# Stalfoes/dqn_mgsc_zoo

Measured on AMD Instinct MI355X. Metric: learner grad-steps/sec at batch=32, 84×84×4 uint8, 1/2/4/8 MI355X, higher is better.
Workload: dtype f32

## Files before the change

### dqn_mgsc_zoo_amd/_native.py

```python

import ctypes
import glob
import hashlib
import os
import threading

_HERE = os.path.dirname(os.path.abspath(__file__))
LIB_PATH = os.environ.get('DQZ_LIB') or os.path.join(_HERE, 'libdqz.so')
HEADER_PATH = os.path.join(os.path.dirname(_HERE), 'include', 'dqz.h')

DQZ_OK = 0
ALGO_DQN = 0
ALGO_DOUBLE = 1
ALGO_PER = 2
NUM_LEAVES = 10
NUM_PHASES = 10
PHASE_NAMES = (
    'conv1_fwd', 'conv2_fwd', 'conv3_fwd', 'fc1_fwd', 'head', 'fc1_dx',
    'conv3_dx+conv2_dx+fc1_dw+conv3_dw+conv2_dw+conv1_dw', 'unused7',
    'unused8', 'update')
FRAME_H = 84
FRAME_W = 84
STACK = 4
FRAME_BYTES = FRAME_H * FRAME_W
# ... 210 lines not shown
        [_vp, ctypes.POINTER(DqzParams), ctypes.POINTER(DqzStore), _i64, _i64,
         _i64, ctypes.c_uint64, _vp, _vp, _vp, _vp, _vp]),
    'dqz_learner_step_opt_per_draw': (
        _int,
        [_vp, ctypes.POINTER(DqzParams), ctypes.POINTER(DqzStore),
         ctypes.POINTER(DqzPerDraw), _vp, _vp, _vp]),
    'dqz_learner_grad': (
        _int,
        [_vp, ctypes.POINTER(DqzParams), ctypes.POINTER(DqzStore), _vp, _vp,
         _vp, _vp],
    ),
    'dqz_learner_outputs': (_int, [_vp, _vp, _vp, _vp, _vp]),
    'dqz_learner_sync_status': (_int, [_vp, _vp]),
    'dqz_learner_debug_stall': (_int, [_vp, _int, ctypes.c_uint]),
    'dqz_learner_debug_backward': (_int, [_vp, _int, _vp]),
    'dqz_learner_debug_sync_words': (_int, [_vp, _vp, _i64, _vp]),
    'dqz_learner_debug_activations': (_int, [_vp, _int] + [_vp] * 10),
    'dqz_per_write_back': (_int, [_vp, _vp, _i64, _vp, ctypes.c_double, _vp, _vp]),
    'dqz_learner_profile': (
        _int,
        [_vp, ctypes.POINTER(DqzParams), ctypes.POINTER(DqzStore), _vp, _vp,
         _int, ctypes.POINTER(ctypes.c_float), _vp],
    ),
    'dqz_forward': (_int, [_vp, _vp, _vp, _int, _vp, _vp]),
    'dqz_forward_slots': (
        _int, [_vp, _vp, ctypes.POINTER(DqzStore), _vp, _int, _int, _vp, _vp]),
    'dqz_act': (
        _int, [_vp, _vp, _vp, _int, ctypes.c_double, ctypes.c_uint64,
               ctypes.c_uint64, _vp, _vp]),
    'dqz_store_put': (
# ... 257 lines not shown
```

### dqn_mgsc_zoo_amd/csrc/common.hpp

```cpp
#pragma once
#include <hip/hip_runtime.h>

#include <cstdarg>
#include <cstdint>
#include <cstdio>
#include <string>

#include "dqz.h"

namespace dqz {

typedef float f32x4 __attribute__((ext_vector_type(4)));

#define DQZ_STR(x) #x
#define DQZ_XSTR(x) DQZ_STR(x)
typedef float f32x16 __attribute__((ext_vector_type(16)));

#ifdef DQZ_STEP_TU
#define DQZ_STEP_KERNEL __global__
#define DQZ_OTHER_KERNEL template <int = 0> __global__
#else
#define DQZ_STEP_KERNEL template <int = 0> __global__
#define DQZ_OTHER_KERNEL __global__
#endif
// ... 100 lines not shown
    const float w = 2.f * u * (-lr) * rs3 * (d2 - c1 * g * (g - m));
    nu = w;
    sq += u * u;
    s1 += gq * w;
  }
  __device__ __forceinline__ float meta2(float g, float m0, float v0, float j, float& sq) const {
    const float m = c1 * g + decay * m0;
    const float v = c1 * (g * g) + decay * v0;
    const float u = (-lr) * (g * rsqrtf(v - m * m + eps));
    sq += u * u;
    return -2.f * u * j;
  }
};

#ifdef DQZ_TRACE
constexpr int TRACE_KERNELS = 24, TRACE_BLOCKS = 4096, TRACE_SLOTS = 4;
static __device__ unsigned long long g_dqz_trace[TRACE_KERNELS * TRACE_BLOCKS * TRACE_SLOTS];
#define DQZ_STAMP(kid, slot)                                                                              \
  do {                                                                                                    \
    if (threadIdx.x == 0) {                                                                               \
      const unsigned bl_ = blockIdx.x + gridDim.x * (blockIdx.y + gridDim.y * blockIdx.z);                \
      if (bl_ < (unsigned)dqz::TRACE_BLOCKS)                                                              \
        dqz::g_dqz_trace[((kid) * dqz::TRACE_BLOCKS + bl_) * dqz::TRACE_SLOTS + (slot)] =                \
            __builtin_amdgcn_s_memrealtime();                                                             \
    }                                                                                                     \
  } while (0)
#else
#define DQZ_STAMP(kid, slot) \
  do {                       \
  } while (0)
#endif
// ... 108 lines not shown
  }
  __device__ __forceinline__ void release_finish(int b, int prior, [[maybe_unused]] int hk = -1) const {
    __builtin_amdgcn_sched_barrier(0);
    if (threadIdx.x == 0 && prior == consumers - 1) {
      __hip_atomic_store(cnt + b * kStride, 0, __ATOMIC_RELAXED, __HIP_MEMORY_SCOPE_AGENT);
      __hip_atomic_store(ack + b * kStride, 0, __ATOMIC_RELAXED, __HIP_MEMORY_SCOPE_AGENT);
    }
    if (hk >= 0) DQZ_STAMP(hk, 3);
  }
  __device__ __forceinline__ void wait_release(int b) const {
    wait(b);
    release_finish(b, release_issue(b));
  }
};

constexpr int kTraceY1 = 20, kTraceY2 = 21, kTraceDy2 = 22, kTraceDy1 = 23;

__device__ __forceinline__ float4 load_sc1_f4(const float4* base, int bytes, int e) {
  typedef unsigned u32x4 __attribute__((ext_vector_type(4)));
  const __amdgpu_buffer_rsrc_t r = __builtin_amdgcn_make_buffer_rsrc((void*)base, 0, bytes, 0x00020000);
  return __builtin_bit_cast(float4, __builtin_amdgcn_raw_buffer_load_b128(r, e * 16, 0, 16));
}

__device__ __forceinline__ float load_sc1_f1(const float* base, int bytes, int e) {
  const __amdgpu_buffer_rsrc_t r = __builtin_amdgcn_make_buffer_rsrc((void*)base, 0, bytes, 0x00020000);
  return __builtin_bit_cast(float, __builtin_amdgcn_raw_buffer_load_b32(r, e * 4, 0, 16));
}

__device__ __forceinline__ void store_sc1_f4(float* base, int bytes, int off, f32x4 v) {
  typedef unsigned u32x4 __attribute__((ext_vector_type(4)));
  const __amdgpu_buffer_rsrc_t r = __builtin_amdgcn_make_buffer_rsrc((void*)base, 0, bytes, 0x00020000);
// ... 26 lines not shown
```

### dqn_mgsc_zoo_amd/csrc/fwd.hpp

```cpp
#pragma once
#include "common.hpp"
#include "conv1.hpp"

namespace dqz {


__device__ __forceinline__ f32x4 mfma4(float a, float b, f32x4 c) {
  return __builtin_amdgcn_mfma_f32_16x16x4f32(a, b, c, 0, 0, 0);
}

__device__ __forceinline__ int red_idx(int row, int col) { return row * 16 + 16 * (row >> 2) + col; }

__device__ __forceinline__ int epi_row(int i) {
  return ((i >> 6) << 4) + (int)((0xFBAE9DC873261540ull >> (4 * ((i >> 2) & 15))) & 15);
}
constexpr int epi_range(int rows) { return (rows + 15) / 16 * 64; }
constexpr int red_rows(int rows) { return rows * 16 + 16 * ((rows + 3) / 4); }

struct LayerFwdArgs {
  const float* in;
  NetZ nz;
  int64_t w_off, b_off;
  int B, Z;
  int linear;
// ... 429 lines not shown
}

constexpr int FC1_S = 7, FC1_KS = FLAT / FC1_S, FC1_KW = FC1_KS / 4;
constexpr int Z_MAX_FC1 = 3;

struct Fc1FwdArgs {
  const float* in;
  NetZ nz;
  int64_t w_off;
  int B, MG;
  float* part;
  TangentDot dot = {nullptr, nullptr, 0};
};

constexpr int FC1_32RW = 32 * 33;
template <bool DOT>
__device__ __forceinline__ void fc1_fwd_block32(const Fc1FwdArgs& a, float* s_red, int i) {
  const int nt = i % (HID / 32);
  const int rest = i / (HID / 32);
  const int s = rest % FC1_S, zm = rest / FC1_S;
  const int z = zm / a.MG, mg = zm % a.MG;
  const int t = threadIdx.x, lane = t & 63, w = t >> 6;
  const int c = lane & 31, h = lane >> 5;
  const int k0 = s * FC1_KS + w * FC1_KW + 4 * h;
  const float* W = a.nz.p[z] + a.w_off + 32 * nt + c;
  constexpr int G = FC1_KW / 8;
  const int row = min(32 * mg + c, a.B - 1);
  const float* x = a.in + ((int64_t)z * a.B + row) * FLAT + k0;
  float wr[G][4];
  float4 av[G];
#pragma unroll
  for (int g = 0; g < G; ++g)
// ... 21 lines not shown
    v[e] = (s_red[k] + s_red[FC1_32RW + k]) + (s_red[2 * FC1_32RW + k] + s_red[3 * FC1_32RW + k]);
  }
  if (DOT) {
    float d = 0.f;
    if (live) {
      const float4 dz = *reinterpret_cast<const float4*>(a.dot.dy + (int64_t)(32 * mg + q) * HID + 32 * nt + c4);
      d = (v[0] * dz.x + v[1] * dz.y) + (v[2] * dz.z + v[3] * dz.w);
    }
    d += __shfl_xor(d, 1, 64);
    d += __shfl_xor(d, 2, 64);
    d += __shfl_xor(d, 4, 64);
    if (live && (t & 7) == 0)
      a.dot.part[(int64_t)(32 * mg + q) * META_DOT_SLOTS + a.dot.slot0 + nt * FC1_S + s] = d;
    return;
  }
  if (live)
    *reinterpret_cast<float4*>(a.part + (((int64_t)z * FC1_S + s) * a.B + 32 * mg + q) * HID + 32 * nt + c4) =
        make_float4(v[0], v[1], v[2], v[3]);
}

inline int fc1_fwd_blocks(int Z, int MG) { return (HID / 32) * FC1_S * Z * MG; }

constexpr int FC1_GEMV_MAXB = 4, FC1_GEMV_KG = FC1_KS / 8;
constexpr int FC1_GEMV_SMEM = FC1_GEMV_MAXB * FC1_KS + 8 * FC1_GEMV_MAXB * 32;
__device__ __forceinline__ void fc1_gemv_block(const Fc1FwdArgs& a, float* smem, int i) {
  const int nt = i % (HID / 32);
  const int rest = i / (HID / 32);
  const int s = rest % FC1_S, z = rest / FC1_S;
  const int t = threadIdx.x, c = t & 31, kg = t >> 5;
  const int B = a.B;
// ... 53 lines not shown
```

### dqn_mgsc_zoo_amd/csrc/head.hpp

```cpp
#pragma once
#include "common.hpp"

namespace dqz {

struct HeadArgs {
  const float* fc1p;
  int S;
  float* h1;
  NetZ nz;
  int64_t b1_off, w2_off, b2_off;
  int Z, B, A, algo, shared_bias, fwd_only;
  const int32_t* slots;
  const int32_t* action;
  const float* reward;
  const float* discount;
  const float* weights;
  const double* per_wb;
  int per_normalize;
  float* per_w_out;
  const float* meta_p;
  const float* meta_logits;
  const int32_t* meta_pos;
  int meta_M;
  float *meta_x_out, *meta_p_out;
// ... 32 lines not shown
  return dqz_action{act, v};
}

__device__ __forceinline__ double wave_max_nonneg(double m) {
  m = fmax(m, dpp_d<0x111>(m));
  m = fmax(m, dpp_d<0x112>(m));
  m = fmax(m, dpp_d<0x114>(m));
  m = fmax(m, dpp_d<0x118>(m));
  m = fmax(m, dpp_d<0x142, 0xa>(m));
  m = fmax(m, dpp_d<0x143, 0xc>(m));
  const long long b = __builtin_bit_cast(long long, m);
  const int lo = __builtin_amdgcn_readlane((int)b, 63), hi = __builtin_amdgcn_readlane((int)(b >> 32), 63);
  return __builtin_bit_cast(double, ((long long)hi << 32) | (unsigned)lo);
}

template <int AMAX, int SMAX, int ZMAX>
__device__ __forceinline__ void head_body(const HeadArgs& h, int b, bool out = true, float* s_dzo = nullptr) {
  DQZ_STAMP(4, 0);
  __shared__ float s_red[8][3 * AMAX];
  __shared__ float s_q[3][AMAX];
  __shared__ float s_rec[5];
  const int n = threadIdx.x, lane = n & 63, wave = n >> 6;
  const int A = h.A, B = h.B, Z = h.Z, S = h.S;
  int a_tm1 = 0;
  float r = 0.f, d = 0.f, w = 1.f, pm = 0.f;
  const bool chain = !h.fwd_only && h.rec == nullptr;
  const int slot = chain ? h.slots[b] : 0;
  float4 rv = make_float4(0.f, 0.f, 0.f, 0.f);
  if (!h.fwd_only && h.rec != nullptr && n == 0) rv = h.rec[b];
  float pv[ZMAX][SMAX], b1v[ZMAX], w2v[ZMAX][AMAX];
#pragma unroll
  for (int z = 0; z < ZMAX; ++z) {
    const int zc = min(z, Z - 1);
    const float* part = h.fc1p + ((int64_t)zc * S * B + b) * HID + n;
#pragma unroll
    for (int s = 0; s < SMAX; ++s) pv[z][s] = part[(int64_t)min(s, S - 1) * B * HID];
    b1v[z] = h.nz.p[zc][h.b1_off + n];
    const float* w2 = h.nz.p[zc] + h.w2_off + n * A;
#pragma unroll
    for (int a = 0; a < AMAX; ++a) w2v[z][a] = w2[min(a, A - 1)];
  }
  constexpr bool kTr = AMAX <= 8;
  constexpr int kPS = HID + 16;
  __shared__ float s_p[kTr ? 3 * AMAX : 1][kTr ? kPS : 1];
  const int K = Z * A, lgT = K <= 16 ? 5 : 4, T = 1 << lgT;
  const int kk = n >> lgT, jj = n & (T - 1);
  const bool qthread = kTr ? (kk < K && jj == 0) : (n < 3 * AMAX && n / AMAX < Z && n % AMAX < A);
  const int zq = kTr ? min(kk / A, 2) : n / AMAX, aq = kTr ? kk % A : n % AMAX;
  float b2v = 0.f;
  {
    const int a2 = h.shared_bias ? 0 : min(aq, A - 1);
    float b2z[ZMAX];
#pragma unroll
    for (int z = 0; z < ZMAX; ++z) b2z[z] = h.nz.p[min(z, Z - 1)][h.b2_off + a2];
    const int zc = min(zq, Z - 1);
#pragma unroll
    for (int z = 0; z < ZMAX; ++z) b2v = zc == z ? b2z[z] : b2v;
  }
  float wper = 1.f;
// ... 41 lines not shown
      d = h.discount[slot];
    } else {
      a_tm1 = __float_as_int(rv.x);
      r = rv.y;
      d = rv.z;
    }
    if (h.weights) w = h.weights[b];
    if (h.per_wb) w = wper;
    if (h.meta_p && !h.meta_logits) pm = h.meta_p[b];
    s_rec[0] = __int_as_float(a_tm1);
    s_rec[1] = r;
    s_rec[2] = d;
    s_rec[3] = w;
    s_rec[4] = pm;
  }
  DQZ_STAMP(4, 1);
  float hz[ZMAX];
#pragma unroll
  for (int z = 0; z < ZMAX; ++z) hz[z] = 0.f;
#pragma unroll
  for (int z = 0; z < ZMAX; ++z) {
    if (z < Z) {
      float acc = b1v[z];
#pragma unroll
      for (int s = 0; s < SMAX; ++s) acc += s < S ? pv[z][s] : 0.f;
      hz[z] = relu(acc);
      if (z == 0) DQZ_STAMP(15, 0);
      if constexpr (kTr) {
#pragma unroll
        for (int a = 0; a < AMAX; ++a)
          if (a < A) s_p[z * A + a][n] = hz[z] * w2v[z][a];
      } else {
#pragma unroll
        for (int a = 0; a < AMAX; ++a) {
          const float sa = wave_sum(hz[z] * w2v[z][a]);
          if (lane == 0) s_red[wave][z * AMAX + a] = sa;
        }
      }
    }
  }
  DQZ_STAMP(15, 1);
  __syncthreads();
  float qv = 0.f;
  if constexpr (kTr) {
    if (kk < K) {
      const float* row = &s_p[kk][jj];
      float a4[4] = {0.f, 0.f, 0.f, 0.f};
      for (int i = 0; i < (HID >> lgT); i += 4) {
#pragma unroll
        for (int u = 0; u < 4; ++u) a4[u] += row[(i + u) << lgT];
      }
      float v = (a4[0] + a4[1]) + (a4[2] + a4[3]);
      v += dpp_f<0xB1>(v);
      v += dpp_f<0x4E>(v);
      v += dpp_f<0x141>(v);
      v += dpp_f<0x140>(v);
      if (T == 32) v += __shfl_xor(v, 16, 64);
      qv = v + b2v;
      if (jj == 0) s_q[zq][aq] = qv;
    }
  } else if (qthread) {
// ... 60 lines not shown
      for (int a = 1; a < AMAX; ++a) wv = a == a_tm1 ? w2v[0][a] : wv;
      DQZ_STAMP(4, 2);
      const float dz = hz[0] > 0.f ? -g * wv : 0.f;
      if (s_dzo) s_dzo[n] = dz;
      if (out) h.dz1[(int64_t)b * HID + n] = dz;
    }
  } else if (h.act_out) {
    __syncthreads();
    if (out && n == 0) {
      const uint4 r = philox4x32(make_uint4((unsigned)h.act_ctr, (unsigned)(h.act_ctr >> 32), (unsigned)b, 0xAC7u),
                                 make_uint2((unsigned)h.act_seed, (unsigned)(h.act_seed >> 32)));
      const double u = ((((uint64_t)r.x << 32) | r.y) >> 11) * 0x1.0p-53;
      h.act_out[b] = eps_greedy(s_q[0], A, h.eps, u);
    }
  }
  if (!out) return;
#pragma unroll
  for (int z = 0; z < ZMAX; ++z)
    if (z < Z) h.h1[((int64_t)z * B + b) * HID + n] = hz[z];
  if (qthread) h.q[((int64_t)zq * B + b) * A + aq] = qv;
  if (h.advance && b == 0 && n == 0)
    __hip_atomic_fetch_add(h.advance, (uint64_t)1, __ATOMIC_RELAXED, __HIP_MEMORY_SCOPE_AGENT);
  DQZ_STAMP(4, 3);
}

template <int AMAX, int SMAX, int ZMAX>
__global__ __launch_bounds__(512) void head_kernel(HeadArgs h) {
  head_body<AMAX, SMAX, ZMAX>(h, blockIdx.x);
}

// ... 2 lines not shown
inline void launch_head_z(const HeadArgs& h, int grid, hipStream_t st) {
  if (h.A <= 8)
    hipLaunchKernelGGL((head_kernel<8, SMAX, ZMAX>), dim3(grid), dim3(HID), 0, st, h);
  else
    hipLaunchKernelGGL((head_kernel<MAXA, SMAX, ZMAX>), dim3(grid), dim3(HID), 0, st, h);
}

inline hipError_t launch_head(const HeadArgs& h, int grid, hipStream_t st) {
  if (h.S > 7 || h.Z < 1 || h.Z > 3) return hipErrorInvalidValue;
  if (h.Z <= 2) {
    launch_head_z<7, 2>(h, grid, st);
  } else {
    launch_head_z<7, 3>(h, grid, st);
  }
  return hipGetLastError();
}
#endif

struct UpdArgs {
  float *th, *mu, *nu;
  int64_t off[10];
  int64_t sz[10];
  const float* p1;
  const float* p2;
  const float* p3;
  int S1, S2, S3;
  const float* h1;
  const float* dz1;
  const float* gq;
  const int32_t* ga;
// ... 316 lines not shown
```

### dqn_mgsc_zoo_amd/csrc/layout.hpp

```cpp
#pragma once
#include <cstddef>
#include <cstdint>

namespace dqz {

constexpr int kWordStride = 64;

struct HandoffWords {
  int64_t cnt, ack;
  int need, consumers;
  bool learner_spin;
};

struct SyncLayout {
  int64_t B;
  constexpr int64_t word(int64_t w) const { return w * kWordStride; }
  constexpr HandoffWords dy2() const { return {word(0), word(B), 8, 16, true}; }
  constexpr HandoffWords fwd_y1(int jobs) const { return {word(2 * B), word(5 * B), 4, jobs, false}; }
  constexpr HandoffWords fwd_y2(int jobs) const { return {word(8 * B), word(11 * B), jobs, jobs, false}; }
  constexpr HandoffWords dy1() const { return {word(14 * B), word(15 * B), 8, 8, true}; }
  constexpr int64_t err() const { return word(16 * B); }
  constexpr int64_t ints() const { return word(16 * B + 3) + 64; }
};

enum MetaWord {
  kMetaReseed,
  kMetaDdot1Cnt,
  kMetaDdot1Ack,
  kMetaAdamEntry,
  kMetaErr,
  kMetaWords
};

struct Carve {
  void** pp;
  int64_t n;
  template <class T>
// ... 15 lines not shown
```

### dqn_mgsc_zoo_amd/csrc/learner_impl.hpp

```cpp
#pragma once
#include <hip/hip_runtime.h>

#include <cstring>

#include "common.hpp"
#include "layout.hpp"
#include "conv1.hpp"
#include "fwd.hpp"
#include "head.hpp"
#include "bwd.hpp"
#include "sampling.hpp"

namespace dqz {

inline void param_layout(int A, int shared_bias, int64_t off[10], int64_t sz[10], int64_t* total) {
  const int64_t sizes[10] = {C1KK * C1CO, C1CO, C2KK * C2CO, C2CO, C3KK * C3CO, C3CO,
                             (int64_t)FLAT * HID, HID, (int64_t)HID * A, shared_bias ? 1 : A};
  int64_t o = 0;
  for (int i = 0; i < 10; ++i) {
    off[i] = o;
    sz[i] = sizes[i];
    o += (sizes[i] + 63) / 64 * 64;
  }
  *total = o;
// ... 1 lines not shown

}

struct dqz_learner {
  dqz_learner_config cfg;
  int Z, shared_bias;
  int64_t off[10], sz[10], total;
  int S_fc1, S2, S3;
  float *y1, *y2, *y3, *fc1p, *h1, *q, *dz1, *dy3, *dy2, *dy1, *p1, *p2, *p3, *td, *loss, *loss_part, *gq, *rec;
  float *w3p, *w2p;
  double* per_wb;
  int32_t* ga;
  int32_t* sync;
  unsigned spin_max = 1u << 24;
  int bwd_chain = -1;
  void* block;
};

namespace dqz {

static_assert(Handoff::kStride == kWordStride, "layout.hpp's word stride is Handoff's");

inline SyncLayout sync_of(const dqz_learner* L) { return SyncLayout{L->cfg.batch}; }
inline Handoff handoff(const dqz_learner* L, const HandoffWords& w) {
  Handoff h{L->sync + w.cnt, L->sync + w.ack, L->sync + sync_of(L).err(), w.need, w.consumers};
  if (w.learner_spin) h.spin_max = L->spin_max;
  return h;
}

inline bool bwd_chain_active(const dqz_learner* L) {
  if (L->cfg.batch > BWD_CHAIN_MAXB) return false;
  return L->bwd_chain < 0 ? L->cfg.batch > 1 : L->bwd_chain != 0;
}

inline int check_store(const dqz_store* S) {
  if (!S || !S->frames || !S->fidx || !S->action || !S->reward || !S->discount)
    return fail(DQZ_ERR_INVALID, "store has a null buffer");
  if (S->capacity < 1) return fail(DQZ_ERR_INVALID, "store capacity must be positive");
  return DQZ_OK;
}

inline int device_view(const void* p, const void** out, const char* what) {
  hipPointerAttribute_t attr;
  if (hipPointerGetAttributes(&attr, p) != hipSuccess) {
    (void)hipGetLastError();
    return fail(DQZ_ERR_INVALID, "%s must be device memory or pinned host memory", what);
  }
// ... 219 lines not shown
```

### dqn_mgsc_zoo_amd/csrc/learner_step.hip

```cpp
#define DQZ_STEP_TU 1
#include <hip/hip_runtime.h>

#include <cstdlib>
#include <cstring>

#include "learner_impl.hpp"

using namespace dqz;

static int g_attr_done = 0;

static int init_kernel_attrs() {
  if (g_attr_done) return DQZ_OK;
  const void* fwd_kernels[] = {(const void*)fwd_conv_kernel<0>, (const void*)fwd_conv_kernel<1>,
                               (const void*)fwd_conv_kernel<2>, (const void*)fwd_conv_kernel<3>,
                               (const void*)fwd_conv_kernel<4>};
  for (const void* k : fwd_kernels)
    DQZ_HIP(hipFuncSetAttribute(k, hipFuncAttributeMaxDynamicSharedMemorySize, (int)kConv1FwdSmem));
  g_attr_done = 1;
  return DQZ_OK;
}

extern "C" {

// ... 13 lines not shown
  if (int rc = init_kernel_attrs()) return rc;
  dqz_learner* L = new dqz_learner();
  L->cfg = *cfg;
  L->Z = cfg->algo == DQZ_ALGO_DQN ? 2 : 3;
  L->shared_bias = cfg->algo == DQZ_ALGO_DQN ? 0 : 1;
  param_layout(cfg->num_actions, L->shared_bias, L->off, L->sz, &L->total);
  const int64_t B = cfg->batch, Z = L->Z, A = cfg->num_actions;
  L->S_fc1 = FC1_S;
  L->S2 = L->S3 = cfg->batch;
  const Carve bufs[] = {
      {&L->y1, Z * B * C1M * C1CO}, {&L->y2, Z * B * C2M * C2CO}, {&L->y3, Z * B * FLAT},
      {&L->fc1p, Z * L->S_fc1 * B * HID}, {&L->h1, Z * B * HID}, {&L->q, Z * B * A},
      {&L->dz1, B * HID}, {&L->dy3, B * FLAT}, {&L->dy2, B * C2M * C2CO}, {&L->dy1, B * C1M * C1CO},
      {&L->p1, B * C1_BLOCKS * (C1KK + 1) * C1CO}, {&L->p2, B * (C2KK + 1) * C2CO}, {&L->p3, B * (C3KK + 1) * C3CO},
      {&L->td, B}, {&L->loss, 1}, {&L->loss_part, B}, {&L->gq, B}, {&L->ga, B}, {&L->rec, 4 * B},
      {&L->sync, SyncLayout{B}.ints()}, {&L->w3p, W3P_N}, {&L->w2p, W2P_N}, {&L->per_wb, 2 * B}};
  const int64_t total = carve(bufs, nullptr);
  if (hipMalloc(&L->block, total * sizeof(float)) != hipSuccess) {
    delete L;
    return fail(DQZ_ERR_HIP, "hipMalloc of %lld bytes failed", (long long)(total * 4));
  }
  if (hipMemset(L->block, 0, total * sizeof(float)) != hipSuccess) {
    (void)hipFree(L->block);
    delete L;
    return fail(DQZ_ERR_HIP, "hipMemset of learner scratch failed");
  }
  carve(bufs, (float*)L->block);
  *out = L;
  return DQZ_OK;
}

// ... 18 lines not shown
        DQZ_HIP(hipEventRecord(pe.e0, st));                                 \
        for (int r_ = 0; r_ < pe.reps; ++r_) {                              \
          __VA_ARGS__;                                                      \
        }                                                                   \
        DQZ_HIP(hipEventRecord(pe.e1, st));                                 \
        DQZ_HIP(hipEventSynchronize(pe.e1));                                \
        float ms_ = 0.f;                                                    \
        (void)hipEventElapsedTime(&ms_, pe.e0, pe.e1);                      \
        if (t_ == 0 || ms_ < best_) best_ = ms_;                            \
      }                                                                     \
      pe.ms[i] = best_ / (float)pe.reps;                                    \
    }                                                                       \
  } while (0)

static int forward_impl(dqz_learner* L, const NetZ& nz, int Z, int B, const Conv1Src& src, hipStream_t st,
                        PhaseEvents pe) {
  FwdArgs a = make_fwd_args(L, nz, Z, B, src);
  Conv1FwdArgs& c1 = a.c1;
  LayerFwdArgs &c2 = a.c2, &c3 = a.c3;
  const int jobs = fwd_conv_jobs(Z * B);
  c2.jobs = c3.jobs = jobs;
  c1.pub = c2.wait = handoff(L, sync_of(L).fwd_y1(jobs));
  c2.pub = c3.wait = handoff(L, sync_of(L).fwd_y2(jobs));
  const dim3 grid(xcd_grid(4, Z * B).x + 2 * xcd_grid(jobs, Z * B).x);
  DQZ_PHASE(0, switch (src.fused) {
    case 1: hipLaunchKernelGGL(fwd_conv_kernel<1>, grid, dim3(256), kConv1FwdSmem, st, c1, c2, c3); break;
    case 2: hipLaunchKernelGGL(fwd_conv_kernel<2>, grid, dim3(256), kConv1FwdSmem, st, c1, c2, c3); break;
    case 3: hipLaunchKernelGGL(fwd_conv_kernel<3>, grid, dim3(256), kConv1FwdSmem, st, c1, c2, c3); break;
    case 4: hipLaunchKernelGGL(fwd_conv_kernel<4>, grid, dim3(256), kConv1FwdSmem, st, c1, c2, c3); break;
    default: hipLaunchKernelGGL(fwd_conv_kernel<0>, grid, dim3(256), kConv1FwdSmem, st, c1, c2, c3); break;
  } DQZ_HIP(hipGetLastError()));
  if (pe.on()) pe.ms[1] = pe.ms[2] = 0.f;

  const Fc1FwdArgs& f1 = a.f1;
  DQZ_PHASE(3, if (B <= FC1_GEMV_MAXB)
                 hipLaunchKernelGGL(fc1_gemv_kernel, dim3(fc1_fwd_blocks(Z, 1)), dim3(256), 0, st, f1);
               else
                 hipLaunchKernelGGL(fc1_fwd32_kernel, dim3(fc1_fwd_blocks(Z, f1.MG)), dim3(256), 0, st, f1);
            DQZ_HIP(hipGetLastError()));
  return DQZ_OK;
}

static HeadArgs make_head(dqz_learner* L, const NetZ& nz, int Z, int B) {
  HeadArgs h{};
  memset(&h, 0, sizeof(h));
  h.fc1p = L->fc1p;
  h.S = L->S_fc1;
  h.h1 = L->h1;
  h.nz = nz;
// ... 49 lines not shown
    if (r.wide->weighted && !r.is_weights)
      return fail(DQZ_ERR_INVALID, "a weighted %s step needs is_weights", d.noun);
    if (r.pd) return fail(DQZ_ERR_INVALID, "the %s head takes no prioritized draw", d.noun);
    if (r.draw || r.sm || r.smx) return fail(DQZ_ERR_INVALID, "the %s head takes no in-launch batch draw", d.noun);
    if (r.meta_p || r.meta_epi || r.meta_sm) return fail(DQZ_ERR_INVALID, "%s", d.no_meta);
    if (r.unit) return fail(DQZ_ERR_INVALID, "%s", d.no_unit);
    if (r.wb) return fail(DQZ_ERR_INVALID, "%s", d.no_wb);
    if (!r.gout) return fail(DQZ_ERR_INVALID, "%s", d.no_fused);
    if (L->cfg.batch == 1) return fail(DQZ_ERR_INVALID, "the %s head needs batch >= 2", d.noun);
    if (L->cfg.algo != (r.wide->double_q ? DQZ_ALGO_DOUBLE : DQZ_ALGO_DQN))
      return fail(DQZ_ERR_INVALID, "the %s head runs on a DQN learner", d.noun);
  }
  return DQZ_OK;
}

int dqz::step_enqueue(dqz_learner* L, const dqz_params* P, const dqz_store* S, const StepRequest& r, void* stream) {
  hipStream_t st = (hipStream_t)stream;
  const PhaseEvents pe = r.pe;
  const PerSampleArgs* const pd = r.pd;
  const int B = L->cfg.batch, Z = L->Z, A = L->cfg.num_actions;
  const NetZ nz{{P->online, P->target, P->online}, {0, 1, 1}};
  Conv1Src fsrc{S->frames, S->fidx, nullptr, nullptr, 0, UniformDraw{}};
  fsrc.action = S->action;
  fsrc.reward = S->reward;
  fsrc.discount = S->discount;
  fsrc.rec = reinterpret_cast<float4*>(L->rec);
  fsrc.xout = r.xout;
  Conv1Src src = fsrc;
  const Batch batch = decode_batch(r, &fsrc);
  fsrc.fused = batch.fused;
  fsrc.slots = src.slots = batch.slots;
  if (pd) fsrc.per.out_wb = L->per_wb;
  if (int rc = forward_impl(L, nz, Z, B, fsrc, st, pe)) return rc;

  Rms rms{};
  if (r.meta_epi) rms = *r.meta_epi;
  rms.lr = L->cfg.learning_rate;
  rms.decay = L->cfg.decay;
  rms.c1 = (float)(1.0 - (double)L->cfg.decay);
  rms.eps = L->cfg.eps;
  rms.gout = r.gout;
  rms.gacc = r.gacc;
  rms.sq_off = 0;

  HeadArgs h = make_head(L, nz, Z, B);
  h.fwd_only = 0;
  h.slots = batch.slots;
  h.action = S->action;
// ... 37 lines not shown
  fb.w2 = P->online + L->off[2];
  fb.w3p = L->w3p;
  fb.w2p = L->w2p;
  if (r.wide) {
    DQZ_PHASE(4, if (int rc = wide_launch(WIDE_OUTPUTS, L, P, r, st)) return rc);
    DQZ_PHASE(8, if (int rc = wide_launch(WIDE_HEAD, L, P, r, st)) return rc);
    const bool rb = r.wide->kind == WIDE_RB;
    if (r.wide->dout || rb) DQZ_PHASE(2, if (int rc = wide_launch(WIDE_DZ1, L, P, r, st)) return rc);
    if (rb)
      DQZ_PHASE(5, if (int rc = wide_launch(WIDE_FC1_DX, L, P, r, st)) return rc);
    else
      DQZ_PHASE(5, hipLaunchKernelGGL(fc1_dx_kernel, dim3(fc1_dx_blocks(B)), dim3(256), 0, st, fb);
                DQZ_HIP(hipGetLastError()));
  } else if (B == 1 && !pe.on()) {
    DQZ_HIP(launch_head_dx1(h, fb, st));
  } else {
    DQZ_PHASE(4, DQZ_HIP(launch_head(h, B, st)));
    DQZ_PHASE(5, hipLaunchKernelGGL(fc1_dx_kernel, dim3(fc1_dx_blocks(B)), dim3(256), 0, st, fb);
              DQZ_HIP(hipGetLastError()));
  }

  Conv3BwdArgs c3b{};
  c3b.dy3 = L->dy3;
  c3b.y2 = L->y2;
  c3b.w3 = P->online + L->off[4];
  c3b.w3p = L->w3p;
  c3b.dy2 = L->dy2;
  c3b.part = L->p3;
  c3b.B = B;
  c3b.sync = handoff(L, sync_of(L).dy2());
// ... 144 lines not shown
    const SyncLayout at = sync_of(L);
    DQZ_HIP(hipDeviceSynchronize());
    DQZ_HIP(hipMemcpy(L->sync + at.dy2().cnt + at.word(sample), &poison, sizeof(poison), hipMemcpyHostToDevice));
  }
  return DQZ_OK;
}

int dqz_learner_debug_backward(dqz_learner* L, int chain, int* active) {
  if (!L) return fail(DQZ_ERR_INVALID, "null learner");
  if (chain < -1 || chain > 1) return fail(DQZ_ERR_INVALID, "chain must be -1, 0 or 1");
  L->bwd_chain = chain;
  if (active) *active = bwd_chain_active(L) ? 1 : 0;
  return DQZ_OK;
}

int dqz_learner_debug_sync_words(dqz_learner* L, int32_t* out, int64_t n, int64_t* total) {
  if (!L) return fail(DQZ_ERR_INVALID, "null learner");
  const int64_t ints = sync_of(L).ints();
  if (total) *total = ints;
  if (n < 0 || n > ints) return fail(DQZ_ERR_INVALID, "n must be in [0, %lld]", (long long)ints);
  if (n > 0 && !out) return fail(DQZ_ERR_INVALID, "null out");
  if (n == 0) return DQZ_OK;
  DQZ_HIP(hipDeviceSynchronize());
  DQZ_HIP(hipMemcpy(out, L->sync, sizeof(int32_t) * n, hipMemcpyDeviceToHost));
  return DQZ_OK;
}

int dqz_learner_outputs(dqz_learner* L, float* q_tm1, float* td, float* loss, void* stream) {
  if (!L) return fail(DQZ_ERR_INVALID, "null learner");
  hipStream_t st = (hipStream_t)stream;
// ... 33 lines not shown
  const ForwardInput in{.from_store = true, .store = S, .slots = slots, .which = which, .q_out = q_out};
  if (int rc = forward_src(L, params, n, in, &src)) return rc;
  return forward_q(L, params, src, which, n, q_out, nullptr, (hipStream_t)stream);
}

int dqz_act(dqz_learner* L, const float* params, const uint8_t* states, int n, double epsilon, uint64_t seed,
            uint64_t counter, dqz_action* out, void* stream) {
  ActorDraw act{epsilon, seed, counter, out};
  Conv1Src src;
  if (int rc = forward_src(L, params, n, {.states = states, .act = &act}, &src)) return rc;
  return forward_q(L, params, src, 0, n, L->q, &act, (hipStream_t)stream);
}

}

#ifdef DQZ_TRACE
extern "C" int dqz_debug_trace(unsigned long long* host_out, int clear) {
  const size_t bytes = sizeof(unsigned long long) * TRACE_KERNELS * TRACE_BLOCKS * TRACE_SLOTS;
  if (host_out) DQZ_HIP(hipMemcpyFromSymbol(host_out, HIP_SYMBOL(g_dqz_trace), bytes));
  if (clear) {
    void* p = nullptr;
    DQZ_HIP(hipGetSymbolAddress(&p, HIP_SYMBOL(g_dqz_trace)));
    DQZ_HIP(hipMemset(p, 0, bytes));
  }
  return DQZ_OK;
}
#endif
```

### dqn_mgsc_zoo_amd/learner.py

```python

import ctypes

import numpy as np
import torch

from dqn_mgsc_zoo_amd import _native
from dqn_mgsc_zoo_amd import networks as networks_lib
from dqn_mgsc_zoo_amd import optim_state

ALGOS = {'dqn': _native.ALGO_DQN, 'double': _native.ALGO_DOUBLE,
         'per': _native.ALGO_PER}


class RMSPropConfig:

  def __init__(self, learning_rate, decay=0.9, eps=1e-8, centered=False):
    self.learning_rate = float(learning_rate)
    self.decay = float(decay)
    self.eps = float(eps)
    self.centered = bool(centered)


def rmsprop(learning_rate, decay=0.9, eps=1e-8, centered=False):
  return RMSPropConfig(learning_rate, decay, eps, centered)
# ... 314 lines not shown
        _native.ptr(self.loss), _native.stream_handle(stream)))
    return self.q_tm1, self.td, self.loss

  def sync_status(self):
    st = ctypes.c_int(0)
    _native.check(_native.lib().dqz_learner_sync_status(self._h, ctypes.byref(st)))
    return st.value

  def debug_stall(self, sample, spin_max=0):
    _native.check(_native.lib().dqz_learner_debug_stall(self._h, int(sample), int(spin_max)))

  def debug_backward(self, chain=-1):
    active = ctypes.c_int(-1)
    _native.check(_native.lib().dqz_learner_debug_backward(
        self._h, int(chain), ctypes.byref(active)))
    return active.value

  def debug_sync_words(self):
    total = ctypes.c_int64(0)
    fn = _native.lib().dqz_learner_debug_sync_words
    _native.check(fn(self._h, None, 0, ctypes.byref(total)))
    out = np.zeros((total.value,), np.int32)
    _native.check(fn(self._h, out.ctypes.data, total.value, None))
    return out

  def fetch_activations(self, z=0, backward=False, stream=None):
    b, a = self.batch_size, self.network.num_actions
    shapes = dict(y1=(b, 20, 20, 32), y2=(b, 9, 9, 64), y3=(b, 7, 7, 64),
                  h1=(b, 512), q=(b, a))
    if backward:
# ... 551 lines not shown
```

### include/dqz.h

```cpp
#ifndef DQZ_H_
#define DQZ_H_

#include <stdint.h>

#ifdef __cplusplus
extern "C" {
#endif

#define DQZ_OK 0
#define DQZ_ERR_INVALID (-1)
#define DQZ_ERR_HIP (-2)
#define DQZ_ERR_UNSUPPORTED (-3)

#define DQZ_ALGO_DQN 0
#define DQZ_ALGO_DOUBLE 1
#define DQZ_ALGO_PER 2

#define DQZ_FRAME_H 84
#define DQZ_FRAME_W 84
#define DQZ_STACK 4
#define DQZ_FRAME_BYTES (DQZ_FRAME_H * DQZ_FRAME_W)
#define DQZ_NUM_LEAVES 10

const char* dqz_last_error(void);
// ... 60 lines not shown
                     const int32_t* slots, const float* is_weights, float* grad_out, void* stream);

#define DQZ_NUM_PHASES 10

int dqz_learner_profile(dqz_learner* learner, const dqz_params* params, const dqz_store* store,
                        const int32_t* slots, const float* is_weights, int iters, float* phase_ms,
                        void* stream);

int dqz_learner_outputs(dqz_learner* learner, float* q_tm1, float* td, float* loss, void* stream);

int dqz_learner_sync_status(dqz_learner* learner, int* status);

int dqz_learner_debug_stall(dqz_learner* learner, int sample, unsigned spin_max);

int dqz_learner_debug_backward(dqz_learner* learner, int chain, int* active);

int dqz_learner_debug_sync_words(dqz_learner* learner, int32_t* out, int64_t n, int64_t* total);

int dqz_learner_debug_activations(dqz_learner* learner, int z, float* y1, float* y2, float* y3, float* h1,
                                  float* q, float* dz1, float* dy3, float* dy2, float* dy1, void* stream);

int dqz_forward(dqz_learner* learner, const float* params, const uint8_t* states, int n,
                float* q_out, void* stream);

int dqz_forward_slots(dqz_learner* learner, const float* params, const dqz_store* store,
                      const int32_t* slots, int n, int which, float* q_out, void* stream);

typedef struct dqz_action {
  int32_t action;
  float value;
// ... 350 lines not shown
```

### profiles/trace_split.py

```python
import collections
import csv
import re
import sys

path = sys.argv[1]
eager = int(sys.argv[2]) if len(sys.argv) > 2 else 3
reps = int(sys.argv[3]) if len(sys.argv) > 3 else 20
rows = collections.defaultdict(list)
for r in csv.DictReader(open(path)):
  m = re.search(r'dqz::(\w+_kernel)', r['Kernel_Name'])
  if m:
    rows[m.group(1)].append((int(r['Start_Timestamp']), int(r['End_Timestamp'])))
print('%-22s %6s %9s %9s' % ('kernel', 'n', 'graph_us', 'b2b_us'))
for k, v in sorted(rows.items()):
  v.sort()
  d = [(e - s) / 1e3 for s, e in v]
  g, p = d[eager:len(d) - reps], d[len(d) - reps:]
  print('%-22s %6d %9.2f %9.2f' % (k, len(d), sum(g) / max(1, len(g)), sum(p) / max(1, len(p))))
```

Baseline: 17200.

## Fuse fc1 forward and head into one kernel with a sharded in-kernel handoff

```diff
diff --git a/dqn_mgsc_zoo_amd/_native.py b/dqn_mgsc_zoo_amd/_native.py
--- a/dqn_mgsc_zoo_amd/_native.py
+++ b/dqn_mgsc_zoo_amd/_native.py
@@ -248,6 +248,7 @@
     'dqz_learner_sync_status': (_int, [_vp, _vp]),
     'dqz_learner_debug_stall': (_int, [_vp, _int, ctypes.c_uint]),
     'dqz_learner_debug_backward': (_int, [_vp, _int, _vp]),
+    'dqz_learner_debug_fc1_head': (_int, [_vp, _int, _vp]),
     'dqz_learner_debug_sync_words': (_int, [_vp, _vp, _i64, _vp]),
     'dqz_learner_debug_activations': (_int, [_vp, _int] + [_vp] * 10),
     'dqz_per_write_back': (_int, [_vp, _vp, _i64, _vp, ctypes.c_double, _vp, _vp]),
diff --git a/dqn_mgsc_zoo_amd/csrc/common.hpp b/dqn_mgsc_zoo_amd/csrc/common.hpp
--- a/dqn_mgsc_zoo_amd/csrc/common.hpp
+++ b/dqn_mgsc_zoo_amd/csrc/common.hpp
@@ -138,7 +138,7 @@
 };
 
 #ifdef DQZ_TRACE
-constexpr int TRACE_KERNELS = 24, TRACE_BLOCKS = 4096, TRACE_SLOTS = 4;
+constexpr int TRACE_KERNELS = 25, TRACE_BLOCKS = 4096, TRACE_SLOTS = 4;
 static __device__ unsigned long long g_dqz_trace[TRACE_KERNELS * TRACE_BLOCKS * TRACE_SLOTS];
 #define DQZ_STAMP(kid, slot)                                                                              \
   do {                                                                                                    \
@@ -277,7 +277,59 @@
   }
 };
 
-constexpr int kTraceY1 = 20, kTraceY2 = 21, kTraceDy2 = 22, kTraceDy1 = 23;
+constexpr int kTraceY1 = 20, kTraceY2 = 21, kTraceDy2 = 22, kTraceDy1 = 23, kTraceFc1H = 24;
+
+struct ShardedHandoff {
+  static constexpr int kStride = Handoff::kStride;
+  int* cnt;
+  int* ack;
+  int* err;
+  int shards;
+  int need, extra;
+  int consumers;
+  unsigned spin_max;
+  __device__ __forceinline__ void arrive(int p) const {
+    asm volatile("s_waitcnt vmcnt(0)" ::: "memory");
+    __syncthreads();
+    if (threadIdx.x == 0)
+      __hip_atomic_fetch_add(cnt + (p & (shards - 1)) * kStride, 1, __ATOMIC_RELAXED, __HIP_MEMORY_SCOPE_AGENT);
+  }
+  __device__ __forceinline__ void wait([[maybe_unused]] int hk = -1) const {
+    if (threadIdx.x < 64) {
+      const int l = min((int)threadIdx.x, shards - 1);
+      const int want = need + (l < extra ? 1 : 0);
+      const int* p = cnt + l * kStride;
+      unsigned spins = 0;
+      while (!__all(__hip_atomic_load(p, __ATOMIC_RELAXED, __HIP_MEMORY_SCOPE_AGENT) >= want)) {
+        __builtin_amdgcn_s_sleep(4);
+        if (++spins > spin_max) {
+          if (threadIdx.x == 0) __hip_atomic_fetch_or(err, 1, __ATOMIC_RELAXED, __HIP_MEMORY_SCOPE_AGENT);
+          break;
+        }
+      }
+    }
+    if (hk >= 0) DQZ_STAMP(hk, 0);
+    __syncthreads();
+    if (hk >= 0) DQZ_STAMP(hk, 1);
+  }
+  __device__ __forceinline__ int release_issue() const {
+    int prior = 0;
+    if (threadIdx.x == 0) {
+      int* p = ack + __builtin_amdgcn_mbcnt_lo(~0u, 0u);
+      prior = __hip_atomic_fetch_add(p, 1, __ATOMIC_RELAXED, __HIP_MEMORY_SCOPE_AGENT);
+    }
+    return prior;
+  }
+  __device__ __forceinline__ void release_finish(int prior, [[maybe_unused]] int hk = -1) const {
+    __builtin_amdgcn_sched_barrier(0);
+    if (threadIdx.x == 0 && prior == consumers - 1) {
+      for (int l = 0; l < shards; ++l)
+        __hip_atomic_store(cnt + l * kStride, 0, __ATOMIC_RELAXED, __HIP_MEMORY_SCOPE_AGENT);
+      __hip_atomic_store(ack, 0, __ATOMIC_RELAXED, __HIP_MEMORY_SCOPE_AGENT);
+    }
+    if (hk >= 0) DQZ_STAMP(hk, 3);
+  }
+};
 
 __device__ __forceinline__ float4 load_sc1_f4(const float4* base, int bytes, int e) {
   typedef unsigned u32x4 __attribute__((ext_vector_type(4)));
diff --git a/dqn_mgsc_zoo_amd/csrc/fwd.hpp b/dqn_mgsc_zoo_amd/csrc/fwd.hpp
--- a/dqn_mgsc_zoo_amd/csrc/fwd.hpp
+++ b/dqn_mgsc_zoo_amd/csrc/fwd.hpp
@@ -467,8 +467,14 @@
 };
 
 constexpr int FC1_32RW = 32 * 33;
-template <bool DOT>
-__device__ __forceinline__ void fc1_fwd_block32(const Fc1FwdArgs& a, float* s_red, int i) {
+template <bool DOT, bool PUB = false>
+__device__ __forceinline__ void fc1_fwd_block32(const Fc1FwdArgs& a, float* s_red, int i,
+                                                const ShardedHandoff* pub = nullptr, int part_bytes = 0) {
+  if (PUB && threadIdx.x >= 256) {
+    __syncthreads();
+    pub->arrive(i);
+    return;
+  }
   const int nt = i % (HID / 32);
   const int rest = i / (HID / 32);
   const int s = rest % FC1_S, zm = rest / FC1_S;
@@ -520,6 +526,13 @@
       a.dot.part[(int64_t)(32 * mg + q) * META_DOT_SLOTS + a.dot.slot0 + nt * FC1_S + s] = d;
     return;
   }
+  if (PUB) {
+    if (live)
+      store_sc1_f4(a.part, part_bytes, 4 * ((((z * FC1_S + s) * a.B + 32 * mg + q) * HID) + 32 * nt + c4),
+                   f32x4{v[0], v[1], v[2], v[3]});
+    pub->arrive(i);
+    return;
+  }
   if (live)
     *reinterpret_cast<float4*>(a.part + (((int64_t)z * FC1_S + s) * a.B + 32 * mg + q) * HID + 32 * nt + c4) =
         make_float4(v[0], v[1], v[2], v[3]);
diff --git a/dqn_mgsc_zoo_amd/csrc/head.hpp b/dqn_mgsc_zoo_amd/csrc/head.hpp
--- a/dqn_mgsc_zoo_amd/csrc/head.hpp
+++ b/dqn_mgsc_zoo_amd/csrc/head.hpp
@@ -1,5 +1,6 @@
 #pragma once
 #include "common.hpp"
+#include "fwd.hpp"
 
 namespace dqz {
 
@@ -70,8 +71,13 @@
   return __builtin_bit_cast(double, ((long long)hi << 32) | (unsigned)lo);
 }
 
-template <int AMAX, int SMAX, int ZMAX>
-__device__ __forceinline__ void head_body(const HeadArgs& h, int b, bool out = true, float* s_dzo = nullptr) {
+template <int AMAX>
+constexpr int head_sp_floats() {
+  return AMAX <= 8 ? 3 * AMAX * (HID + 16) : 1;
+}
+template <int AMAX, int SMAX, int ZMAX, bool FUSED = false>
+__device__ __forceinline__ void head_body(const HeadArgs& h, int b, bool out = true, float* s_dzo = nullptr,
+                                          float* s_ext = nullptr, const ShardedHandoff* wt = nullptr) {
   DQZ_STAMP(4, 0);
   __shared__ float s_red[8][3 * AMAX];
   __shared__ float s_q[3][AMAX];
@@ -88,9 +94,11 @@
 #pragma unroll
   for (int z = 0; z < ZMAX; ++z) {
     const int zc = min(z, Z - 1);
-    const float* part = h.fc1p + ((int64_t)zc * S * B + b) * HID + n;
-#pragma unroll
-    for (int s = 0; s < SMAX; ++s) pv[z][s] = part[(int64_t)min(s, S - 1) * B * HID];
+    if constexpr (!FUSED) {
+      const float* part = h.fc1p + ((int64_t)zc * S * B + b) * HID + n;
+#pragma unroll
+      for (int s = 0; s < SMAX; ++s) pv[z][s] = part[(int64_t)min(s, S - 1) * B * HID];
+    }
     b1v[z] = h.nz.p[zc][h.b1_off + n];
     const float* w2 = h.nz.p[zc] + h.w2_off + n * A;
 #pragma unroll
@@ -98,7 +106,10 @@
   }
   constexpr bool kTr = AMAX <= 8;
   constexpr int kPS = HID + 16;
-  __shared__ float s_p[kTr ? 3 * AMAX : 1][kTr ? kPS : 1];
+  static_assert(!kTr || head_sp_floats<AMAX>() == 3 * AMAX * kPS, "head_sp_floats is s_p's size");
+  __shared__ float s_p_own[!FUSED && kTr ? 3 * AMAX : 1][!FUSED && kTr ? kPS : 1];
+  float(*const s_p)[!FUSED && kTr ? kPS : 1] = s_p_own;
+  float(*const s_px)[kPS] = reinterpret_cast<float(*)[kPS]>(s_ext);
   const int K = Z * A, lgT = K <= 16 ? 5 : 4, T = 1 << lgT;
   const int kk = n >> lgT, jj = n & (T - 1);
   const bool qthread = kTr ? (kk < K && jj == 0) : (n < 3 * AMAX && n / AMAX < Z && n % AMAX < A);
@@ -170,6 +181,18 @@
     s_rec[3] = w;
     s_rec[4] = pm;
   }
+  [[maybe_unused]] int ack = 0;
+  if constexpr (FUSED) {
+    wt->wait(kTraceFc1H);
+    const int bytes = Z * S * B * HID * (int)sizeof(float);
+#pragma unroll
+    for (int z = 0; z < ZMAX; ++z)
+#pragma unroll
+      for (int s = 0; s < SMAX; ++s)
+        pv[z][s] = load_sc1_f1(h.fc1p, bytes, ((min(z, Z - 1) * S + min(s, S - 1)) * B + b) * HID + n);
+    DQZ_STAMP(kTraceFc1H, 2);
+    ack = wt->release_issue();
+  }
   DQZ_STAMP(4, 1);
   float hz[ZMAX];
 #pragma unroll
@@ -185,7 +208,7 @@
       if constexpr (kTr) {
 #pragma unroll
         for (int a = 0; a < AMAX; ++a)
-          if (a < A) s_p[z * A + a][n] = hz[z] * w2v[z][a];
+          if (a < A) (FUSED ? s_px[z * A + a][n] : s_p[z * A + a][n]) = hz[z] * w2v[z][a];
       } else {
 #pragma unroll
         for (int a = 0; a < AMAX; ++a) {
@@ -200,7 +223,7 @@
   float qv = 0.f;
   if constexpr (kTr) {
     if (kk < K) {
-      const float* row = &s_p[kk][jj];
+      const float* row = FUSED ? &s_px[kk][jj] : &s_p[kk][jj];
       float a4[4] = {0.f, 0.f, 0.f, 0.f};
       for (int i = 0; i < (HID >> lgT); i += 4) {
 #pragma unroll
@@ -291,6 +314,7 @@
       h.act_out[b] = eps_greedy(s_q[0], A, h.eps, u);
     }
   }
+  if constexpr (FUSED) wt->release_finish(ack, kTraceFc1H);
   if (!out) return;
 #pragma unroll
   for (int z = 0; z < ZMAX; ++z)
@@ -323,6 +347,20 @@
     launch_head_z<7, 3>(h, grid, st);
   }
   return hipGetLastError();
+}
+
+template <int AMAX, int SMAX, int ZMAX>
+__global__ __launch_bounds__(512) void fc1_head_kernel(Fc1FwdArgs f, HeadArgs h, ShardedHandoff y, int nfc1) {
+  constexpr int kLds = 4 * FC1_32RW > head_sp_floats<AMAX>() ? 4 * FC1_32RW : head_sp_floats<AMAX>();
+  __shared__ __attribute__((aligned(16))) float smem[kLds];
+  const int i = blockIdx.x;
+  if (i < nfc1) {
+    DQZ_STAMP(3, 0);
+    fc1_fwd_block32<false, true>(f, smem, i, &y, h.Z * h.S * h.B * HID * (int)sizeof(float));
+    DQZ_STAMP(3, 3);
+    return;
+  }
+  head_body<AMAX, SMAX, ZMAX, true>(h, i - nfc1, true, nullptr, smem, &y);
 }
 #endif
 
diff --git a/dqn_mgsc_zoo_amd/csrc/layout.hpp b/dqn_mgsc_zoo_amd/csrc/layout.hpp
--- a/dqn_mgsc_zoo_amd/csrc/layout.hpp
+++ b/dqn_mgsc_zoo_amd/csrc/layout.hpp
@@ -12,15 +12,22 @@
   bool learner_spin;
 };
 
+constexpr int kFc1HeadShards = 64;
+struct ShardedWords {
+  int64_t cnt, ack;
+};
+
 struct SyncLayout {
   int64_t B;
+  int64_t tail = 0;
   constexpr int64_t word(int64_t w) const { return w * kWordStride; }
   constexpr HandoffWords dy2() const { return {word(0), word(B), 8, 16, true}; }
   constexpr HandoffWords fwd_y1(int jobs) const { return {word(2 * B), word(5 * B), 4, jobs, false}; }
   constexpr HandoffWords fwd_y2(int jobs) const { return {word(8 * B), word(11 * B), jobs, jobs, false}; }
   constexpr HandoffWords dy1() const { return {word(14 * B), word(15 * B), 8, 8, true}; }
   constexpr int64_t err() const { return word(16 * B); }
-  constexpr int64_t ints() const { return word(16 * B + 3) + 64; }
+  constexpr ShardedWords fc1_head() const { return {word(16 * B + 4), word(16 * B + 4 + kFc1HeadShards)}; }
+  constexpr int64_t ints() const { return word(16 * B + 3 + tail) + 64; }
 };
 
 enum MetaWord {
diff --git a/dqn_mgsc_zoo_amd/csrc/learner_impl.hpp b/dqn_mgsc_zoo_amd/csrc/learner_impl.hpp
--- a/dqn_mgsc_zoo_amd/csrc/learner_impl.hpp
+++ b/dqn_mgsc_zoo_amd/csrc/learner_impl.hpp
@@ -39,6 +39,7 @@
   int32_t* sync;
   unsigned spin_max = 1u << 24;
   int bwd_chain = -1;
+  int fc1_head = -1;
   void* block;
 };
 
@@ -46,7 +47,7 @@
 
 static_assert(Handoff::kStride == kWordStride, "layout.hpp's word stride is Handoff's");
 
-inline SyncLayout sync_of(const dqz_learner* L) { return SyncLayout{L->cfg.batch}; }
+inline SyncLayout sync_of(const dqz_learner* L) { return SyncLayout{L->cfg.batch, kFc1HeadShards + 1}; }
 inline Handoff handoff(const dqz_learner* L, const HandoffWords& w) {
   Handoff h{L->sync + w.cnt, L->sync + w.ack, L->sync + sync_of(L).err(), w.need, w.consumers};
   if (w.learner_spin) h.spin_max = L->spin_max;
@@ -56,6 +57,20 @@
 inline bool bwd_chain_active(const dqz_learner* L) {
   if (L->cfg.batch > BWD_CHAIN_MAXB) return false;
   return L->bwd_chain < 0 ? L->cfg.batch > 1 : L->bwd_chain != 0;
+}
+
+constexpr bool kFc1HeadDefault = true;
+inline bool fc1_head_active(const dqz_learner* L) {
+  if (L->cfg.batch <= FC1_GEMV_MAXB) return false;
+  return L->fc1_head < 0 ? kFc1HeadDefault : L->fc1_head != 0;
+}
+
+inline ShardedHandoff fc1_head_handoff(const dqz_learner* L, int nfc1, int B) {
+  int shards = 8;
+  while (shards < kFc1HeadShards && nfc1 > 32 * shards) shards *= 2;
+  const ShardedWords w = sync_of(L).fc1_head();
+  return ShardedHandoff{L->sync + w.cnt, L->sync + w.ack, L->sync + sync_of(L).err(), shards,
+                        nfc1 / shards,   nfc1 % shards,   B,                          L->spin_max};
 }
 
 inline int check_store(const dqz_store* S) {
diff --git a/dqn_mgsc_zoo_amd/csrc/learner_step.hip b/dqn_mgsc_zoo_amd/csrc/learner_step.hip
--- a/dqn_mgsc_zoo_amd/csrc/learner_step.hip
+++ b/dqn_mgsc_zoo_amd/csrc/learner_step.hip
@@ -51,7 +51,7 @@
       {&L->dz1, B * HID}, {&L->dy3, B * FLAT}, {&L->dy2, B * C2M * C2CO}, {&L->dy1, B * C1M * C1CO},
       {&L->p1, B * C1_BLOCKS * (C1KK + 1) * C1CO}, {&L->p2, B * (C2KK + 1) * C2CO}, {&L->p3, B * (C3KK + 1) * C3CO},
       {&L->td, B}, {&L->loss, 1}, {&L->loss_part, B}, {&L->gq, B}, {&L->ga, B}, {&L->rec, 4 * B},
-      {&L->sync, SyncLayout{B}.ints()}, {&L->w3p, W3P_N}, {&L->w2p, W2P_N}, {&L->per_wb, 2 * B}};
+      {&L->sync, sync_of(L).ints()}, {&L->w3p, W3P_N}, {&L->w2p, W2P_N}, {&L->per_wb, 2 * B}};
   const int64_t total = carve(bufs, nullptr);
   if (hipMalloc(&L->block, total * sizeof(float)) != hipSuccess) {
     delete L;
@@ -100,7 +100,7 @@
   } while (0)
 
 static int forward_impl(dqz_learner* L, const NetZ& nz, int Z, int B, const Conv1Src& src, hipStream_t st,
-                        PhaseEvents pe) {
+                        PhaseEvents pe, Fc1FwdArgs* f1_out = nullptr) {
   FwdArgs a = make_fwd_args(L, nz, Z, B, src);
   Conv1FwdArgs& c1 = a.c1;
   LayerFwdArgs &c2 = a.c2, &c3 = a.c3;
@@ -119,6 +119,10 @@
   if (pe.on()) pe.ms[1] = pe.ms[2] = 0.f;
 
   const Fc1FwdArgs& f1 = a.f1;
+  if (f1_out) {
+    *f1_out = f1;
+    return DQZ_OK;
+  }
   DQZ_PHASE(3, if (B <= FC1_GEMV_MAXB)
                  hipLaunchKernelGGL(fc1_gemv_kernel, dim3(fc1_fwd_blocks(Z, 1)), dim3(256), 0, st, f1);
                else
@@ -198,6 +202,9 @@
   return DQZ_OK;
 }
 
+static hipError_t launch_fc1_head(const Fc1FwdArgs& f, const HeadArgs& h, const ShardedHandoff& y, int nfc1,
+                                  hipStream_t st);
+
 int dqz::step_enqueue(dqz_learner* L, const dqz_params* P, const dqz_store* S, const StepRequest& r, void* stream) {
   hipStream_t st = (hipStream_t)stream;
   const PhaseEvents pe = r.pe;
@@ -215,7 +222,9 @@
   fsrc.fused = batch.fused;
   fsrc.slots = src.slots = batch.slots;
   if (pd) fsrc.per.out_wb = L->per_wb;
-  if (int rc = forward_impl(L, nz, Z, B, fsrc, st, pe)) return rc;
+  const bool fused_head = fc1_head_active(L) && !r.wide && !pe.on();
+  Fc1FwdArgs f1{};
+  if (int rc = forward_impl(L, nz, Z, B, fsrc, st, pe, fused_head ? &f1 : nullptr)) return rc;
 
   Rms rms{};
   if (r.meta_epi) rms = *r.meta_epi;
@@ -283,6 +292,11 @@
                 DQZ_HIP(hipGetLastError()));
   } else if (B == 1 && !pe.on()) {
     DQZ_HIP(launch_head_dx1(h, fb, st));
+  } else if (fused_head) {
+    const int nfc1 = fc1_fwd_blocks(Z, f1.MG);
+    DQZ_HIP(launch_fc1_head(f1, h, fc1_head_handoff(L, nfc1, B), nfc1, st));
+    hipLaunchKernelGGL(fc1_dx_kernel, dim3(fc1_dx_blocks(B)), dim3(256), 0, st, fb);
+    DQZ_HIP(hipGetLastError());
   } else {
     DQZ_PHASE(4, DQZ_HIP(launch_head(h, B, st)));
     DQZ_PHASE(5, hipLaunchKernelGGL(fc1_dx_kernel, dim3(fc1_dx_blocks(B)), dim3(256), 0, st, fb);
@@ -457,6 +471,14 @@
   return DQZ_OK;
 }
 
+int dqz_learner_debug_fc1_head(dqz_learner* L, int mode, int* active) {
+  if (!L) return fail(DQZ_ERR_INVALID, "null learner");
+  if (mode < -1 || mode > 1) return fail(DQZ_ERR_INVALID, "mode must be -1, 0 or 1");
+  L->fc1_head = mode;
+  if (active) *active = fc1_head_active(L) ? 1 : 0;
+  return DQZ_OK;
+}
+
 int dqz_learner_debug_sync_words(dqz_learner* L, int32_t* out, int64_t n, int64_t* total) {
   if (!L) return fail(DQZ_ERR_INVALID, "null learner");
   const int64_t ints = sync_of(L).ints();
@@ -520,6 +542,24 @@
 
 }
 
+static hipError_t launch_fc1_head(const Fc1FwdArgs& f, const HeadArgs& h, const ShardedHandoff& y, int nfc1,
+                                  hipStream_t st) {
+  if (h.S != FC1_S || h.Z < 1 || h.Z > 3) return hipErrorInvalidValue;
+  const dim3 grid(nfc1 + h.B), block(HID);
+  if (h.Z <= 2) {
+    if (h.A <= 8)
+      hipLaunchKernelGGL((fc1_head_kernel<8, 7, 2>), grid, block, 0, st, f, h, y, nfc1);
+    else
+      hipLaunchKernelGGL((fc1_head_kernel<MAXA, 7, 2>), grid, block, 0, st, f, h, y, nfc1);
+  } else {
+    if (h.A <= 8)
+      hipLaunchKernelGGL((fc1_head_kernel<8, 7, 3>), grid, block, 0, st, f, h, y, nfc1);
+    else
+      hipLaunchKernelGGL((fc1_head_kernel<MAXA, 7, 3>), grid, block, 0, st, f, h, y, nfc1);
+  }
+  return hipGetLastError();
+}
+
 #ifdef DQZ_TRACE
 extern "C" int dqz_debug_trace(unsigned long long* host_out, int clear) {
   const size_t bytes = sizeof(unsigned long long) * TRACE_KERNELS * TRACE_BLOCKS * TRACE_SLOTS;
diff --git a/dqn_mgsc_zoo_amd/learner.py b/dqn_mgsc_zoo_amd/learner.py
--- a/dqn_mgsc_zoo_amd/learner.py
+++ b/dqn_mgsc_zoo_amd/learner.py
@@ -352,6 +352,12 @@
     active = ctypes.c_int(-1)
     _native.check(_native.lib().dqz_learner_debug_backward(
         self._h, int(chain), ctypes.byref(active)))
+    return active.value
+
+  def debug_fc1_head(self, mode=-1):
+    active = ctypes.c_int(-1)
+    _native.check(_native.lib().dqz_learner_debug_fc1_head(
+        self._h, int(mode), ctypes.byref(active)))
     return active.value
 
   def debug_sync_words(self):
diff --git a/include/dqz.h b/include/dqz.h
--- a/include/dqz.h
+++ b/include/dqz.h
@@ -98,6 +98,8 @@
 int dqz_learner_debug_stall(dqz_learner* learner, int sample, unsigned spin_max);
 
 int dqz_learner_debug_backward(dqz_learner* learner, int chain, int* active);
+
+int dqz_learner_debug_fc1_head(dqz_learner* learner, int mode, int* active);
 
 int dqz_learner_debug_sync_words(dqz_learner* learner, int32_t* out, int64_t n, int64_t* total);
 
diff --git a/profiles/trace_split.py b/profiles/trace_split.py
--- a/profiles/trace_split.py
+++ b/profiles/trace_split.py
@@ -12,8 +12,18 @@
   if m:
     rows[m.group(1)].append((int(r['Start_Timestamp']), int(r['End_Timestamp'])))
 print('%-22s %6s %9s %9s' % ('kernel', 'n', 'graph_us', 'b2b_us'))
+graph_us = {}
 for k, v in sorted(rows.items()):
   v.sort()
   d = [(e - s) / 1e3 for s, e in v]
-  g, p = d[eager:len(d) - reps], d[len(d) - reps:]
-  print('%-22s %6d %9.2f %9.2f' % (k, len(d), sum(g) / max(1, len(g)), sum(p) / max(1, len(p))))
+  if k == 'fc1_head_kernel':
+    g, p = d[eager:], []
+  elif k in ('fc1_fwd32_kernel', 'head_kernel') and 'fc1_head_kernel' in rows:
+    g, p = [], d
+  else:
+    g, p = d[eager:len(d) - reps], d[len(d) - reps:]
+  graph_us[k] = sum(g) / max(1, len(g))
+  print('%-22s %6d %9.2f %9.2f' % (k, len(d), graph_us[k], sum(p) / max(1, len(p))))
+STEP = ('fwd_conv_kernel', 'fc1_fwd32_kernel', 'head_kernel', 'fc1_head_kernel', 'fc1_dx_kernel', 'bwd_bc_kernel',
+        'update_kernel')
+print('step kernels, graph-averaged sum: %.2f us' % sum(graph_us.get(k, 0.0) for k in STEP))
```

Measured after the change: 17190, median of 2. About the same (-0.1%).
